# Audio-WestlakeU/FullSubNet

Measured on NVIDIA H100. Metric: frames_per_sec, higher is better.
Workload: dtype f16x3(hi+lo split, fp32-class)xf32acc

## Files before the change

### fullsubnet_b200/csrc/fsn_subband_tc.cu

```cuda
#include <cuda_fp16.h>
#include <stdlib.h>
#include <string.h>

#include "fsn_internal.cuh"
#include "fsn_tc_ptx.cuh"
#include "fsn_wgmma.cuh"

namespace fsn {
namespace tc {

using namespace ptx;

constexpr int NB = 32;
constexpr int KB = 64;
constexpr int KS = 32;
constexpr int US = 64;
constexpr int W_SUB = US * KS * 2;
constexpr int W_TILE = 4 * W_SUB;
constexpr int S_KBLK = NB * KB * 2;
constexpr int X_BLK = NB * KS * 2;
constexpr int MAX_STAGES = 4;
constexpr int MAX_MT = 3;
constexpr int OUT_T = 8;
constexpr int NTHREADS = 128 + 128 * MAX_MT;

struct PackedLayout {
  int H, MT, nkb0, nkb1, parts;
  size_t tiles0, tiles1;
  size_t off_bias, off_fcw, off_fcb, bytes;
};

__host__ __device__ inline PackedLayout packed_layout(int H, bool x3) {
  PackedLayout L;
  L.H = H; L.MT = H / 128;
  L.nkb0 = 1 + H / KS; L.nkb1 = 2 * H / KS;
  L.parts = x3 ? 2 : 1;
  L.tiles0 = (size_t)L.MT * L.nkb0 * L.parts;
  L.tiles1 = (size_t)L.MT * L.nkb1 * L.parts;
  L.off_bias = 2 * (L.tiles0 + L.tiles1) * W_TILE;
  L.off_fcw = L.off_bias + (size_t)2 * 4 * H * sizeof(float);
  L.off_fcb = L.off_fcw + (size_t)2 * H * sizeof(float);
  L.bytes = L.off_fcb + 256;
  return L;
}

__global__ void pack_kernel(const float* __restrict__ wih0, const float* __restrict__ whh0,
                            const float* __restrict__ wih1, const float* __restrict__ whh1,
                            const float* __restrict__ bih0, const float* __restrict__ bhh0,
                            const float* __restrict__ bih1, const float* __restrict__ bhh1,
                            const float* __restrict__ fcw, const float* __restrict__ fcb, int H, int Ksb, int x3,
                            int fc_out, uint8_t* __restrict__ out) {
  const PackedLayout L = packed_layout(H, x3 != 0);
  const size_t per_half = L.tiles0 + L.tiles1;
  const size_t total = 2 * per_half * 4 * US * 4;
  for (size_t i = blockIdx.x * (size_t)blockDim.x + threadIdx.x; i < total; i += (size_t)gridDim.x * blockDim.x) {
    const int c = (int)(i & 3);
    const int r = (int)((i >> 2) & (US - 1));
    const int g = (int)((i >> 8) & 3);
    const size_t st_abs = i >> 10;
    const int half = (int)(st_abs / per_half);
    size_t st = st_abs - half * per_half;
    const int layer = st >= L.tiles0;
    if (layer) st -= L.tiles0;
    const int part = (int)(st % L.parts);
    st /= L.parts;
    const int nkb = layer ? L.nkb1 : L.nkb0;
    const int kb = (int)(st % nkb);
    const int m = (int)(st / nkb);
    const int wrow = g * H + (half * L.MT + m) * US + r;
    __half v[8];
#pragma unroll
    for (int e = 0; e < 8; ++e) {
      const int kk = c * 8 + e;
      float w = 0.f;
      if (layer == 0) {
        if (kb == 0) { if (kk < Ksb) w = wih0[(size_t)wrow * Ksb + kk]; }
        else w = whh0[(size_t)wrow * H + (kb - 1) * KS + kk];
      } else {
        const int k = kb * KS + kk;
        w = (k < H) ? wih1[(size_t)wrow * H + k] : whh1[(size_t)wrow * H + (k - H)];
      }
      const __half hi = __float2half_rn(w);
      v[e] = part ? __float2half_rn(w - __half2float(hi)) : hi;
    }
    uint8_t* dst = out + st_abs * W_TILE + g * W_SUB + swz64_off(r, c * 8);
    *reinterpret_cast<uint4*>(dst) = *reinterpret_cast<const uint4*>(v);
  }
  float* bias = reinterpret_cast<float*>(out + L.off_bias);
  float* pfcw = reinterpret_cast<float*>(out + L.off_fcw);
  float* pfcb = reinterpret_cast<float*>(out + L.off_fcb);
  for (int i = blockIdx.x * blockDim.x + threadIdx.x; i < 4 * H; i += gridDim.x * blockDim.x) {
    bias[i] = bih0[i] + bhh0[i];
    bias[4 * H + i] = bih1[i] + bhh1[i];
  }
  for (int i = blockIdx.x * blockDim.x + threadIdx.x; i < 2 * H; i += gridDim.x * blockDim.x)
    pfcw[i] = (i < fc_out * H) ? fcw[i] : 0.f;
  if (blockIdx.x == 0 && threadIdx.x < 2) pfcb[threadIdx.x] = ((int)threadIdx.x < fc_out) ? fcb[threadIdx.x] : 0.f;
}

struct Smem {
  uint32_t w, x, h0, h1, lo, fcw, fcp, outst, rows, bars, total;
};
__host__ __device__ inline Smem smem_plan(int H, int stages, bool x3) {
  Smem s;
  const int nkh = H / KB;
  uint32_t o = 0;
  s.w = o; o += stages * W_TILE;
  s.x = o; o += 2 * X_BLK;
  s.h0 = o; o += 2 * nkh * S_KBLK;
  s.h1 = o; o += nkh * S_KBLK;
  s.lo = o; o += x3 ? (o - s.x) : 0;
  s.fcw = o; o += 4 * MAX_MT * 2 * NB * 4;
  s.fcp = o; o += 2 * 2 * NB * 4;
  s.outst = o; o += NB * 2 * OUT_T * 4;
  s.rows = o; o += NB * 16;
  s.bars = o; o += 256;
  s.total = o;
  return s;
}

struct Bars {
  uint64_t w_full[MAX_STAGES], w_empty[MAX_STAGES];
  uint64_t x_full[2], x_empty[2];
  uint64_t h0_ready[2], h0_empty[2];
  uint64_t h1_ready, h1_empty, fc_done;
  uint64_t l1_done;
  uint64_t fcp_full[2], fcp_empty[2];
  uint64_t turn[MAX_MT];
};
static_assert(sizeof(Bars) <= 256, "barrier block too large");

struct RowInfo {
  int src_b, src_f;
  float scale;
  int out_idx;
};

struct KArgs {
  const uint8_t* packed;
  const float* magT; const float* fbT; const float* inv2;
  const float* unit_scale;
  float* crm;
  int R, F, Tp, la, T, Ns, Nf, H, Ksb, act, Fsub, stages, cluster;
  int src_T, shrink;
  RowMap map;
  long long* stamps;
  int stamp_ctas, stamp_its;
};

enum ProbeField {
  PF_T_BEGIN = 0,
  PF_T_MMA0 = 1,
  PF_T_MMA1 = 2,
  PF_T_END = 3,
  PF_OPERAND = 4,
  PF_TURN = 5,
  PF_W_FULL = 6,
  PF_WAIT_GROUP = 7,
  PF_GROUP_LAT = 8,
  PF_STAGES = 9,
  PF_CELL = 10,
  PF_L1_DONE = 11,
  PF_H1_EMPTY = 12,
  PF_H0_EMPTY = 13,
  PF_FC_DONE = 14,
  PF_GT_BEGIN = 15,
  PROBE_FIELDS = 16
};
constexpr int PROBE_SLOTS = MAX_MT + 1;
static_assert(PROBE_FIELDS == FSN_SB_PROBE_FIELDS && PROBE_SLOTS == FSN_SB_PROBE_SLOTS,
              "probe record layout differs from fsn_b200.h (and fullsubnet_b200/_lib.py)");

__device__ __forceinline__ long long globaltimer() {
  uint64_t t;
  asm volatile("mov.u64 %0, %%globaltimer;" : "=l"(t));
  return (long long)t;
}

__device__ __forceinline__ float act_apply(float v, int act) {
  switch (act) {
    case FSN_ACT_RELU: return fmaxf(v, 0.f);
    case FSN_ACT_TANH: return tanhf(v);
    case FSN_ACT_RELU6: return fminf(fmaxf(v, 0.f), 6.f);
    default: return v;
  }
}
template <bool X3> __device__ __forceinline__ float sg(float x) { return X3 ? 1.0f / (1.0f + expf(-x)) : fast_sigmoid(x); }
template <bool X3> __device__ __forceinline__ float th(float x) { return X3 ? 1.0f - 2.0f / (1.0f + expf(2.0f * x)) : fast_tanh(x); }

__device__ __forceinline__ void release_stage(uint32_t bar, uint32_t pred, uint32_t local, uint32_t remote,
                                              uint32_t rank) {
  mbar_arrive_elect_if(bar, pred & local);
  mbar_arrive_remote_elect_if(bar, rank, pred & remote);
}

template <bool X3, bool PROBE>
__global__ void __launch_bounds__(NTHREADS, 1) sb_lstm_tc_kernel(const __grid_constant__ KArgs a) {
  constexpr int PARTS = X3 ? 2 : 1;
  long long pt = 0;
  auto mark = [&]() -> uint32_t {
    if constexpr (PROBE) {
      const long long n = clock64();
      const uint32_t d = (uint32_t)(n - pt);
      pt = n;
      return d;
    } else {
      return 0u;
    }
  };
  auto record = [&](int it, int layer, int slot) -> long long* {
    return a.stamps + ((((size_t)blockIdx.x * a.stamp_its + it) * 2 + layer) * PROBE_SLOTS + slot) * PROBE_FIELDS;
  };
  const bool probe_cta = PROBE && (int)blockIdx.x < a.stamp_ctas;
  extern __shared__ uint8_t smem_raw[];
  uint8_t* smem = smem_raw + ((1024u - (smem_u32(smem_raw) & 1023u)) & 1023u);
  const int H = a.H;
  const int MT = H / 128;
  const int nkh = H / KB;
  const int STAGES = a.stages;
  const int CL = a.cluster;
  const uint32_t cl_rank = cluster_ctarank();
  const int half = (int)(cl_rank & 1u);
  const uint32_t peer = cl_rank ^ 1u;
  const uint16_t cl_mask = (uint16_t)((0x55u & ((1u << (2 * CL)) - 1u)) << half);
  const Smem sp = smem_plan(H, STAGES, X3);
  const uint32_t LO = sp.lo - sp.x;
  const PackedLayout PL = packed_layout(H, X3);
  Bars& bars = *reinterpret_cast<Bars*>(smem + sp.bars);
  RowInfo* rows = reinterpret_cast<RowInfo*>(smem + sp.rows);
  float* fc_part = reinterpret_cast<float*>(smem + sp.fcw);
  float* fcp = reinterpret_cast<float*>(smem + sp.fcp);
  float* outst = reinterpret_cast<float*>(smem + sp.outst);
  const int warp = threadIdx.x >> 5, lane = threadIdx.x & 31;
  const int row0 = (blockIdx.x >> 1) * NB;
  const int Tp = a.Tp;

  if (threadIdx.x == 0) {
    for (int s = 0; s < STAGES; ++s) { mbar_init(&bars.w_full[s], 1); mbar_init(&bars.w_empty[s], CL); }
    for (int i = 0; i < 2; ++i) {
      mbar_init(&bars.x_full[i], 1); mbar_init(&bars.x_empty[i], 4 * MT);
      mbar_init(&bars.h0_ready[i], 5 * MT);
      mbar_init(&bars.h0_empty[i], MT);
      mbar_init(&bars.fcp_full[i], 1); mbar_init(&bars.fcp_empty[i], 1);
    }
    mbar_init(&bars.h1_ready, 5 * MT);
    mbar_init(&bars.h1_empty, MT);
    mbar_init(&bars.fc_done, 1);
    mbar_init(&bars.l1_done, 4 * MT);
    for (int m = 0; m < MAX_MT; ++m) mbar_init(&bars.turn[m], 4);
    asm volatile("fence.mbarrier_init.release.cluster;" ::: "memory");
  }
  if (threadIdx.x < NB) {
    RowInfo ri;
    const int r = row0 + threadIdx.x;
    ri.src_b = -1; ri.src_f = 0; ri.scale = 0.f; ri.out_idx = 0;
    if (r < a.R) {
      row_to_unit(a.map, r, ri.src_b, ri.src_f);
      ri.scale = a.inv2[ri.src_b];
      const int bq = r / a.Fsub, fq = r - bq * a.Fsub;
      ri.out_idx = bq * 2 * a.Fsub + fq;
    }
    rows[threadIdx.x] = ri;
  }
  {
    uint4* z = reinterpret_cast<uint4*>(smem + sp.x);
    const int n16 = (sp.fcw - sp.x) / 16;
    for (int i = threadIdx.x; i < n16; i += blockDim.x) z[i] = make_uint4(0, 0, 0, 0);
  }
  fence_proxy_async_smem();
  __syncthreads();
  cluster_sync_all();

  if (warp < 4) {
    asm volatile("setmaxnreg.dec.sync.aligned.u32 56;");
  if (warp == 0) {
    const uint8_t* stream = a.packed + (size_t)half * (PL.tiles0 + PL.tiles1) * W_TILE;
    uint32_t stage = 0, phase = 0;
    for (int it = 0; it <= Tp; ++it) {
      const size_t t_begin = (it < Tp) ? 0 : PL.tiles0;
      const size_t t_end = (it >= 1) ? PL.tiles0 + PL.tiles1 : PL.tiles0;
      const uint8_t* src = stream + t_begin * W_TILE;
      long long p_t0 = 0, p_g0 = 0;
      uint32_t p_empty = 0;
      if constexpr (PROBE) { p_g0 = globaltimer(); p_t0 = clock64(); pt = p_t0; }
      for (size_t tile = t_begin; tile < t_end; ++tile, src += W_TILE) {
        mark();
        mbar_wait_cta<false>(&bars.w_empty[stage], phase ^ 1);
        p_empty += mark();
        if (elect_one()) {
          mbar_expect_tx(&bars.w_full[stage], W_TILE);
          if (CL == 1) {
            bulk_g2s(smem + sp.w + stage * W_TILE, src, W_TILE, &bars.w_full[stage]);
          } else {
            const uint32_t slice = W_TILE / CL, off = (cl_rank >> 1) * slice;
            bulk_g2s_mc(smem + sp.w + stage * W_TILE + off, src + off, slice, &bars.w_full[stage], cl_mask);
          }
        }
        __syncwarp();
        if (++stage == (uint32_t)STAGES) { stage = 0; phase ^= 1; }
      }
      if (probe_cta && it < a.stamp_its && lane == 0) {
        long long* r = record(it, 0, MAX_MT);
        r[PF_T_BEGIN] = p_t0; r[PF_T_END] = clock64(); r[PF_OPERAND] = p_empty;
        r[PF_STAGES] = (long long)(t_end - t_begin); r[PF_GT_BEGIN] = p_g0;
      }
    }
  } else if (warp == 2) {
    const int nmag = 2 * a.Ns + 1;
    for (int t = 0; t < Tp; ++t) {
      mbar_wait_cta<true>(&bars.x_empty[t & 1], ((t >> 1) & 1) ^ 1);
      uint8_t* xb = smem + sp.x + (t & 1) * X_BLK;
      int f0 = t, f1 = t + 1;
      if (a.shrink > 1 && t > 0) { f0 = 1 + (t - 1) * a.shrink; f1 = min(f0 + a.shrink, a.src_T); }
      const float wmean = 1.0f / (float)(f1 - f0);
#pragma unroll 4
      for (int n = 0; n < NB; ++n) {
        const RowInfo ri = rows[n];
        float v = 0.f;
        if (ri.src_b >= 0 && lane < a.Ksb) {
          const int col = (lane < nmag) ? reflect_idx(ri.src_f + lane - a.Ns, a.F)
                                        : reflect_idx(ri.src_f + (lane - nmag) - a.Nf, a.F);
          const float* src = (lane < nmag) ? a.magT : a.fbT;
          if (a.shrink <= 1) {
            v = src[((size_t)ri.src_b * a.src_T + t) * a.F + col];
            v *= a.unit_scale ? a.unit_scale[(size_t)t * a.R + row0 + n] : ri.scale;
          } else {
            for (int fr = f0; fr < f1; ++fr) v += src[((size_t)ri.src_b * a.src_T + fr) * a.F + col];
            v *= wmean * (a.unit_scale ? a.unit_scale[(size_t)t * a.R + row0 + n] : ri.scale);
          }
        }
        const __half hi = __float2half_rn(v);
        *reinterpret_cast<__half*>(xb + swz64_off(n, lane)) = hi;
        if (X3) *reinterpret_cast<__half*>(xb + LO + swz64_off(n, lane)) = __float2half_rn(v - __half2float(hi));
      }
      fence_proxy_async_smem();
      __syncwarp();
      if (lane == 0) mbar_arrive(&bars.x_full[t & 1]);
    }
  } else if (warp == 3) {
    const float fcb0 = half ? 0.f : reinterpret_cast<const float*>(a.packed + PL.off_fcb)[0];
    const float fcb1 = half ? 0.f : reinterpret_cast<const float*>(a.packed + PL.off_fcb)[1];
    const RowInfo ri = rows[lane];
    int staged = 0, t_stage0 = 0;
    for (int t = 0; t < Tp; ++t) {
      mbar_wait_cta<true>(&bars.h1_ready, t & 1);
      float s0 = fcb0, s1 = fcb1;
      if (t >= a.la) {
        for (int w = 0; w < 4 * MT; ++w) {
          s0 += fc_part[(w * 2 + 0) * NB + lane];
          s1 += fc_part[(w * 2 + 1) * NB + lane];
        }
      }
      __syncwarp();
      if (lane == 0) mbar_arrive(&bars.fc_done);
      if (t < a.la) continue;
      const int u = t - a.la, b = u & 1;
      float* pb = fcp + b * 2 * NB;
      if (half) {
        mbar_wait<true>(&bars.fcp_empty[b], ((u >> 1) & 1) ^ 1);
        st_remote_f32(pb + lane, peer, s0);
        st_remote_f32(pb + NB + lane, peer, s1);
        __syncwarp();
        if (lane == 0) mbar_arrive_cluster(&bars.fcp_full[b], peer);
        continue;
      }
      mbar_wait<true>(&bars.fcp_full[b], (u >> 1) & 1);
      s0 += pb[lane];
      s1 += pb[NB + lane];
      __syncwarp();
      if (lane == 0) mbar_arrive_cluster(&bars.fcp_empty[b], peer);
      if (staged == 0) t_stage0 = u;
      outst[(lane * 2 + 0) * OUT_T + staged] = act_apply(s0, a.act);
      outst[(lane * 2 + 1) * OUT_T + staged] = act_apply(s1, a.act);
      ++staged;
      if (staged == OUT_T || t == Tp - 1) {
        if (ri.src_b >= 0) {
#pragma unroll
          for (int o = 0; o < 2; ++o) {
            float* dst = a.crm + ((size_t)ri.out_idx + (size_t)o * a.Fsub) * a.T + t_stage0;
            for (int i = 0; i < staged; ++i) dst[i] = outst[(lane * 2 + o) * OUT_T + i];
          }
        }
        staged = 0;
      }
    }
  }
  } else {
    asm volatile("setmaxnreg.inc.sync.aligned.u32 152;");
    const int m = __shfl_sync(0xffffffffu, (warp - 4) >> 2, 0);
    const int q = __shfl_sync(0xffffffffu, warp & 3, 0);
    const int s = half * MT + m;
    if (m < MT) {
      const float* bias_g = reinterpret_cast<const float*>(a.packed + PL.off_bias);
      const float* fcw = reinterpret_cast<const float*>(a.packed + PL.off_fcw);
      float* my_part = fc_part + (size_t)(warp - 4) * 2 * NB;
      float c0[16], c1[16];
#pragma unroll
      for (int i = 0; i < 16; ++i) c0[i] = c1[i] = 0.f;
      const uint32_t a_lo0 = wg::desc_lo(smem_u32(smem + sp.w));
      const uint32_t w_full0 = smem_u32(&bars.w_full[0]), w_empty0 = smem_u32(&bars.w_empty[0]);
      const uint32_t turn_next = smem_u32(&bars.turn[m + 1 < MT ? m + 1 : 0]);
      const uint32_t rel_local = CL == 1 && q == 0, rel_remote = CL > 1 && q < CL;
      const uint32_t rel_rank = 2 * q + half;
      int h0_seen = 0, h1_seen = 0, turns = 0;
      bool first_block = true;
      size_t tile_base = 0;
      for (int it = 0; it <= Tp; ++it) {
        for (int layer = 0; layer < 2; ++layer) {
          const int t = it - layer;
          if (t < 0 || t >= Tp) continue;
          long long p_t0 = 0, p_g0 = 0, p_mma0 = 0, p_mma1 = 0, p_commit = 0, p_commit_prev = 0;
          uint32_t p_opnd = 0, p_turn = 0, p_wfull = 0, p_wgw = 0, p_lat = 0, p_cell = 0, p_l1 = 0, p_h1e = 0, p_h0e = 0,
                   p_fc = 0;
          if constexpr (PROBE) { p_g0 = globaltimer(); p_t0 = clock64(); pt = p_t0; }
          if (layer == 0) {
            mbar_wait_cta<false>(&bars.x_full[t & 1], (t >> 1) & 1);
            for (; h0_seen < t; ++h0_seen) mbar_wait_cta<false>(&bars.h0_ready[h0_seen & 1], (h0_seen >> 1) & 1);
          } else {
            for (; h0_seen < t + 1; ++h0_seen) mbar_wait_cta<false>(&bars.h0_ready[h0_seen & 1], (h0_seen >> 1) & 1);
            for (; h1_seen < t; ++h1_seen) mbar_wait_cta<false>(&bars.h1_ready, h1_seen & 1);
          }
          p_opnd += mark();
          const uint32_t x_addr = smem_u32(smem + sp.x + (t & 1) * X_BLK);
          const uint32_t h0_cur = smem_u32(smem + sp.h0 + (t & 1) * nkh * S_KBLK);
          const uint32_t h0_prev = smem_u32(smem + sp.h0 + ((t + 1) & 1) * nkh * S_KBLK);
          const uint32_t h1_prev = smem_u32(smem + sp.h1);
          const int nkb = layer ? PL.nkb1 : PL.nkb0;
          const size_t first = tile_base + (layer ? ((it < Tp) ? PL.tiles0 : 0) : 0) + (size_t)m * nkb * PARTS;
          float acc[4][16];
#pragma unroll
          for (int g = 0; g < 4; ++g) {
#pragma unroll
            for (int i = 0; i < 16; ++i) acc[g][i] = 0.f;
            wg::fence_operand(acc[g]);
          }
          int prev_stage = -1;
          if (m > 0 || !first_block) { mbar_wait_cta<false>(&bars.turn[m], turns & 1); ++turns; }
          first_block = false;
          p_turn += mark();
          p_mma0 = pt;
          int stage = __shfl_sync(0xffffffffu, (int)(first % (size_t)STAGES), 0);
          uint32_t wphase = __shfl_sync(0xffffffffu, (uint32_t)((first / (size_t)STAGES) & 1), 0);
          auto issue_stage = [&](int part, uint32_t bd, uint32_t b_hi, uint32_t ends_block) {
            mark();
            mbar_wait_cta_warp(w_full0 + 8 * stage, wphase);
            p_wfull += mark();
            mbar_arrive_elect_if(turn_next, ends_block);
            wg::fence();
            const uint32_t ad = a_lo0 + stage * (W_TILE >> 4);
#pragma unroll
            for (int kk = 0; kk < 2; ++kk)
#pragma unroll
              for (int g = 0; g < 4; ++g) {
                const uint32_t a_off = g * (W_SUB >> 4) + kk * 2;
                wg::mma_f16_n32_w(acc[g], ad, a_off, wg::DESC_SW64_HI, bd, kk * 2, b_hi);
                if (X3 && part == 0) wg::mma_f16_n32_w(acc[g], ad, a_off, wg::DESC_SW64_HI, bd, (LO >> 4) + kk * 2, b_hi);
              }
            wg::commit();
            if constexpr (PROBE) p_commit = clock64();
            mark();
            wg::wait<1>();
            p_wgw += mark();
            if constexpr (PROBE) {
              if (prev_stage >= 0) p_lat += (uint32_t)(pt - p_commit_prev);
              p_commit_prev = p_commit;
            }
            release_stage(w_empty0 + 8 * prev_stage, prev_stage >= 0, rel_local, rel_remote, rel_rank);
            prev_stage = stage;
            if (++stage == STAGES) { stage = 0; wphase ^= 1; }
          };
          if (layer == 0) {
#pragma unroll
            for (int part = 0; part < PARTS; ++part) issue_stage(part, wg::desc_lo(x_addr), wg::DESC_SW64_HI, 0u);
          }
          const int nseg = layer ? 2 : 1;
          int seg = 0;
          do {
            uint32_t bd = wg::desc_lo(layer == 0 ? h0_prev : seg == 0 ? h0_cur : h1_prev);
            int kb = 0;
            do {
              const uint32_t ends_block = seg == nseg - 1 && kb == nkh - 1;
#pragma unroll
              for (int part = 0; part < PARTS; ++part) issue_stage(part, bd, wg::DESC_SW128_HI, 0u);
#pragma unroll
              for (int part = 0; part < PARTS; ++part)
                issue_stage(part, bd + (64 >> 4), wg::DESC_SW128_HI, part == PARTS - 1 ? ends_block : 0u);
              bd += S_KBLK >> 4;
            } while (++kb < nkh);
          } while (++seg < nseg);
          mark();
          wg::wait<0>();
#pragma unroll
          for (int g = 0; g < 4; ++g) wg::fence_operand(acc[g]);
          p_wgw += mark();
          if constexpr (PROBE) { p_lat += (uint32_t)(pt - p_commit_prev); p_mma1 = pt; }
          release_stage(w_empty0 + 8 * prev_stage, 1u, rel_local, rel_remote, rel_rank);
          if (lane == 0) mbar_arrive(layer ? &bars.l1_done : &bars.x_empty[t & 1]);
          if (layer == 1 && lane == 0) {
            if (q == 2) mbar_arrive_remote(&bars.h0_empty[t & 1], peer);
            if (q == 3) mbar_arrive_remote(&bars.h1_empty, peer);
          }
          p_cell += mark();
          if (layer == 1 && t >= 1) mbar_wait_cta<false>(&bars.fc_done, (t - 1) & 1);
          p_fc += mark();
          float fsum[2][8];
#pragma unroll
          for (int i = 0; i < 16; ++i) fsum[i >> 3][i & 7] = 0.f;
          __half hv[2][8];
          __half lv[2][8];
          uint8_t* hb = smem + (layer ? sp.h1 : sp.h0 + (t & 1) * nkh * S_KBLK) + s * S_KBLK;
#pragma unroll
          for (int hh = 0; hh < 2; ++hh) {
            const int u = s * US + 16 * q + (lane >> 2) + 8 * hh;
            const float* bl = bias_g + (layer ? 4 * H : 0);
            const float bi = bl[u], bff = bl[H + u], bg = bl[2 * H + u], bo = bl[3 * H + u];
            const float w0 = fcw[u], w1 = fcw[H + u];
#pragma unroll
            for (int j = 0; j < 4; ++j)
#pragma unroll
              for (int e = 0; e < 2; ++e) {
                const int ri = 4 * j + 2 * hh + e;
                const int ci = hh * 8 + j * 2 + e;
                const float cp = layer ? c1[ci] : c0[ci];
                const float cn = sg<X3>(acc[1][ri] + bff) * cp + sg<X3>(acc[0][ri] + bi) * th<X3>(acc[2][ri] + bg);
                if (layer) c1[ci] = cn; else c0[ci] = cn;
                const float h = sg<X3>(acc[3][ri] + bo) * th<X3>(cn);
                const __half hi = __float2half_rn(h);
                hv[hh][j * 2 + e] = hi;
                lv[hh][j * 2 + e] = __float2half_rn(h - __half2float(hi));
                if (layer) { fsum[0][j * 2 + e] += h * w0; fsum[1][j * 2 + e] += h * w1; }
              }
          }
          if (layer == 1) {
#pragma unroll
            for (int o = 0; o < 2; ++o)
#pragma unroll
              for (int r = 0; r < 8; ++r) {
                float v = fsum[o][r];
                v += __shfl_xor_sync(0xffffffffu, v, 4);
                v += __shfl_xor_sync(0xffffffffu, v, 8);
                v += __shfl_xor_sync(0xffffffffu, v, 16);
                fsum[o][r] = v;
              }
            if (lane < 4) {
#pragma unroll
              for (int o = 0; o < 2; ++o)
#pragma unroll
                for (int r = 0; r < 8; ++r) my_part[o * NB + 8 * (r >> 1) + 2 * lane + (r & 1)] = fsum[o][r];
            }
            p_cell += mark();
            mbar_wait_cta<false>(&bars.l1_done, t & 1);
            p_l1 += mark();
            mbar_wait_cta<false>(&bars.h1_empty, t & 1);
            p_h1e += mark();
          } else if (t >= 2) {
            p_cell += mark();
            mbar_wait_cta<false>(&bars.h0_empty[t & 1], ((t - 2) >> 1) & 1);
            p_h0e += mark();
          }
#pragma unroll
          for (int hh = 0; hh < 2; ++hh) {
            const int u = 16 * q + (lane >> 2) + 8 * hh;
            uint8_t* ub = hb + (u & 7) * 2;
            const int chunk = u >> 3;
#pragma unroll
            for (int j = 0; j < 4; ++j)
#pragma unroll
              for (int e = 0; e < 2; ++e) {
                const int n = 8 * j + 2 * (lane & 3) + e;
                uint8_t* p = ub + (n >> 3) * 1024 + (n & 7) * 128 + ((chunk ^ (n & 7)) << 4);
                *reinterpret_cast<__half*>(p) = hv[hh][j * 2 + e];
                if (X3) *reinterpret_cast<__half*>(p + LO) = lv[hh][j * 2 + e];
              }
          }
          fence_proxy_async_smem();
          __syncwarp();
          uint64_t* ready = layer ? &bars.h1_ready : &bars.h0_ready[t & 1];
          if (lane == 0) mbar_arrive(ready);
          named_sync(1 + m, 128);
          if (q == 0 && lane == 0) {
            mbar_arrive_expect_tx_remote(ready, peer, PARTS * S_KBLK);
            bulk_s2s_remote(hb, S_KBLK, ready, peer);
            if (X3) bulk_s2s_remote(hb + LO, S_KBLK, ready, peer);
          }
          if constexpr (PROBE) {
            p_cell += mark();
            if (probe_cta && it < a.stamp_its && q == 0 && lane == 0) {
              long long* r = record(it, layer, m);
              r[PF_T_BEGIN] = p_t0; r[PF_T_MMA0] = p_mma0; r[PF_T_MMA1] = p_mma1; r[PF_T_END] = pt;
              r[PF_OPERAND] = p_opnd; r[PF_TURN] = p_turn; r[PF_W_FULL] = p_wfull; r[PF_WAIT_GROUP] = p_wgw;
              r[PF_GROUP_LAT] = p_lat; r[PF_STAGES] = nkb * PARTS; r[PF_CELL] = p_cell; r[PF_L1_DONE] = p_l1;
              r[PF_H1_EMPTY] = p_h1e; r[PF_H0_EMPTY] = p_h0e; r[PF_FC_DONE] = p_fc; r[PF_GT_BEGIN] = p_g0;
            }
          }
        }
        tile_base += ((it < Tp) ? PL.tiles0 : 0) + ((it >= 1) ? PL.tiles1 : 0);
      }
    }
  }

  __syncthreads();
  cluster_sync_all();
}

}

static int sb_ksb(const fsn_model_desc* d) { return (2 * d->sb_num_neighbors + 1) + (2 * d->fb_num_neighbors + 1); }

static bool sb_tc_shape_ok(int H, int Ksb) { return H % 128 == 0 && H / 128 <= tc::MAX_MT && H >= 128 && Ksb <= tc::KS; }

bool sb_tc_supported(const fsn_model_desc* d) {
  if (d->cell_type != FSN_CELL_LSTM) return false;
  return sb_tc_shape_ok(d->sb_hidden, sb_ksb(d));
}

size_t sb_tc_packed_bytes_raw(int H, bool x3) { return tc::packed_layout(H, x3).bytes; }

size_t sb_tc_packed_bytes(const fsn_model_desc* d) {
  if (!sb_tc_supported(d)) return 0;
  return sb_tc_packed_bytes_raw(d->sb_hidden, d->precision == FSN_PREC_F16X3_TC);
}

int sb_tc_pack_raw(const fsn_seq_weights* sb, int H, int Ksb, int fc_out, void* packed, cudaStream_t st, bool x3) {
  FSN_REQUIRE(sb_tc_shape_ok(H, Ksb), FSN_ERR_UNSUPPORTED,
              "the fp16 tensor-core LSTM stack needs a hidden size in {128,256,384} and an input width <= 32");
  int dev = 0, sms = 132;
  cudaGetDevice(&dev);
  cudaDeviceGetAttribute(&sms, cudaDevAttrMultiProcessorCount, dev);
  tc::pack_kernel<<<sms * 4, 256, 0, st>>>(sb->w_ih[0], sb->w_hh[0], sb->w_ih[1], sb->w_hh[1], sb->b_ih[0], sb->b_hh[0],
                                           sb->b_ih[1], sb->b_hh[1], sb->fc_w, sb->fc_b, H, Ksb, x3 ? 1 : 0, fc_out,
                                           (uint8_t*)packed);
  FSN_CHECK_LAUNCH("sb pack_kernel");
  return FSN_OK;
}

int sb_tc_pack(const fsn_model_desc* d, const fsn_seq_weights* sb, void* packed, cudaStream_t st) {
  FSN_REQUIRE(sb_tc_supported(d), FSN_ERR_UNSUPPORTED,
              "FSN_PREC_F16_TC / FSN_PREC_F16X3_TC need sb_hidden in {128,256,384} and sub-band input width <= 32");
  return sb_tc_pack_raw(sb, d->sb_hidden, sb_ksb(d), 2, packed, st, d->precision == FSN_PREC_F16X3_TC);
}

template <bool X3, bool PROBE = false>
static int sb_tc_config(int H, int stages, int cluster, int pairs, cudaStream_t st, cudaLaunchConfig_t& cfg,
                        cudaLaunchAttribute* attr) {
  const tc::Smem sp = tc::smem_plan(H, stages, X3);
  const size_t smem = sp.total + 1024;
  int rc = check_cuda(cudaFuncSetAttribute(tc::sb_lstm_tc_kernel<X3, PROBE>, cudaFuncAttributeMaxDynamicSharedMemorySize,
                                           (int)smem), "sb_lstm_tc smem attr");
  if (rc) return rc;
// ... 145 lines not shown
```

### fullsubnet_b200/csrc/fsn_tc_ptx.cuh

```cuda
#pragma once
#include <cuda_fp16.h>
#include <stdint.h>
#include <stdio.h>

namespace fsn {
namespace ptx {

__device__ __forceinline__ uint32_t smem_u32(const void* p) { return (uint32_t)__cvta_generic_to_shared(p); }

__device__ __forceinline__ uint32_t cluster_ctarank() {
  uint32_t r;
  asm volatile("mov.u32 %0, %%cluster_ctarank;" : "=r"(r));
  return r;
}
__device__ __forceinline__ uint32_t mapa(uint32_t addr, uint32_t rank) {
  uint32_t r;
  asm volatile("mapa.shared::cluster.u32 %0, %1, %2;" : "=r"(r) : "r"(addr), "r"(rank));
  return r;
}
__device__ __forceinline__ void cluster_sync_all() {
  asm volatile("barrier.cluster.arrive.release.aligned;\n\tbarrier.cluster.wait.acquire.aligned;" ::: "memory");
}
__device__ __forceinline__ bool elect_one() {
  uint32_t pred;
  asm volatile(
      "{\n\t.reg .pred p;\n\t"
      "elect.sync _|p, 0xffffffff;\n\t"
      "selp.b32 %0, 1, 0, p;\n\t}"
      : "=r"(pred));
  return pred != 0;
}

__device__ __forceinline__ void mbar_init(uint64_t* bar, uint32_t count) {
  asm volatile("mbarrier.init.shared::cta.b64 [%0], %1;" ::"r"(smem_u32(bar)), "r"(count));
}
__device__ __forceinline__ void mbar_expect_tx(uint64_t* bar, uint32_t bytes) {
  asm volatile("mbarrier.arrive.expect_tx.shared::cta.b64 _, [%0], %1;" ::"r"(smem_u32(bar)), "r"(bytes) : "memory");
}
__device__ __forceinline__ void mbar_arrive_cluster(uint64_t* bar, uint32_t rank) {
  asm volatile("mbarrier.arrive.release.cluster.shared::cluster.b64 _, [%0];" ::"r"(mapa(smem_u32(bar), rank))
               : "memory");
}
__device__ __forceinline__ void mbar_arrive_cluster_relaxed(uint64_t* bar, uint32_t rank) {
  asm volatile("mbarrier.arrive.relaxed.cluster.shared::cluster.b64 _, [%0];" ::"r"(mapa(smem_u32(bar), rank))
               : "memory");
}
__device__ __forceinline__ void fence_release_cluster() { asm volatile("fence.acq_rel.cluster;" ::: "memory"); }
__device__ __forceinline__ bool mbar_try_wait(uint64_t* bar, uint32_t parity) {
  uint32_t ok;
  asm volatile(
      "{\n\t.reg .pred p;\n\t"
      "mbarrier.try_wait.parity.acquire.cluster.shared::cta.b64 p, [%1], %2;\n\t"
      "selp.b32 %0, 1, 0, p;\n\t}"
      : "=r"(ok)
      : "r"(smem_u32(bar)), "r"(parity)
      : "memory");
  return ok != 0;
}
__device__ __forceinline__ bool mbar_test_wait(uint64_t* bar, uint32_t parity) {
  uint32_t ok;
  asm volatile(
      "{\n\t.reg .pred p;\n\t"
      "mbarrier.test_wait.parity.acquire.cluster.shared::cta.b64 p, [%1], %2;\n\t"
      "selp.b32 %0, 1, 0, p;\n\t}"
      : "=r"(ok)
      : "r"(smem_u32(bar)), "r"(parity)
      : "memory");
  return ok != 0;
}
template <bool RELAXED>
__device__ __forceinline__ void mbar_wait(uint64_t* bar, uint32_t parity) {
  uint32_t spins = 0;
  while (!mbar_try_wait(bar, parity)) {
    if (RELAXED) __nanosleep(64);
    if (++spins > (RELAXED ? (1u << 24) : (1u << 27))) asm volatile("trap;");
  }
}

__device__ __forceinline__ void mbar_wait_mma(uint64_t* bar, uint32_t parity) {
  uint32_t spins = 0;
  while (!mbar_try_wait(bar, parity))
    if (++spins > (1u << 27)) asm volatile("trap;");
}

__device__ __forceinline__ bool mbar_try_wait_cta(uint64_t* bar, uint32_t parity) {
  uint32_t ok;
  asm volatile(
      "{\n\t.reg .pred p;\n\t"
      "mbarrier.try_wait.parity.acquire.cta.shared::cta.b64 p, [%1], %2;\n\t"
      "selp.b32 %0, 1, 0, p;\n\t}"
      : "=r"(ok)
      : "r"(smem_u32(bar)), "r"(parity)
      : "memory");
  return ok != 0;
}
template <bool SLEEP>
__device__ __forceinline__ void mbar_wait_cta(uint64_t* bar, uint32_t parity) {
  uint32_t spins = 0;
  while (!mbar_try_wait_cta(bar, parity)) {
    if (SLEEP) __nanosleep(64);
    if (++spins > (SLEEP ? (1u << 24) : (1u << 27))) asm volatile("trap;");
  }
}
__device__ __forceinline__ void mbar_wait_cta_warp(uint32_t bar, uint32_t parity) {
  asm volatile(
      "{\n\t.reg .pred p;\n\t.reg .b32 n;\n\t"
      "mov.b32 n, 0;\n"
      "WAIT:\n\t"
      "mbarrier.try_wait.parity.acquire.cta.shared::cta.b64 p, [%0], %1;\n\t"
      "vote.sync.all.pred p, p, 0xffffffff;\n\t"
      "@p bra.uni DONE;\n\t"
      "add.u32 n, n, 1;\n\t"
      "setp.gt.u32 p, n, 134217728;\n\t"
      "@p trap;\n\t"
      "bra.uni WAIT;\n"
      "DONE:\n\t}"
      ::"r"(bar), "r"(parity)
      : "memory");
}
__device__ __forceinline__ void mbar_arrive_elect_if(uint32_t bar, uint32_t pred) {
  asm volatile(
      "{\n\t.reg .pred e, p;\n\t"
      "elect.sync _|e, 0xffffffff;\n\t"
      "setp.ne.and.b32 p, %1, 0, e;\n\t"
      "@p mbarrier.arrive.shared::cta.b64 _, [%0];\n\t}"
      ::"r"(bar), "r"(pred)
      : "memory");
}
__device__ __forceinline__ void mbar_arrive_remote_elect_if(uint32_t bar, uint32_t rank, uint32_t pred) {
  asm volatile(
      "{\n\t.reg .pred e, p;\n\t.reg .b32 r;\n\t"
      "elect.sync _|e, 0xffffffff;\n\t"
      "setp.ne.and.b32 p, %2, 0, e;\n\t"
      "@p mapa.shared::cluster.u32 r, %0, %1;\n\t"
      "@p mbarrier.arrive.shared::cluster.b64 _, [r];\n\t}"
      ::"r"(bar), "r"(rank), "r"(pred)
      : "memory");
}
__device__ __forceinline__ void fence_proxy_async_smem() { asm volatile("fence.proxy.async.shared::cta;" ::: "memory"); }
__device__ __forceinline__ void mbar_arrive_remote(uint64_t* bar, uint32_t rank) {
  asm volatile("mbarrier.arrive.shared::cluster.b64 _, [%0];" ::"r"(mapa(smem_u32(bar), rank)) : "memory");
}
__device__ __forceinline__ void mbar_arrive_expect_tx_remote(uint64_t* bar, uint32_t rank, uint32_t bytes) {
  asm volatile("mbarrier.arrive.expect_tx.shared::cluster.b64 _, [%0], %1;" ::"r"(mapa(smem_u32(bar), rank)), "r"(bytes)
               : "memory");
}
__device__ __forceinline__ void bulk_s2s_remote(const void* src, uint32_t bytes, uint64_t* bar, uint32_t rank) {
  const uint32_t s = smem_u32(src);
  asm volatile("cp.async.bulk.shared::cluster.shared::cta.mbarrier::complete_tx::bytes [%0], [%1], %2, [%3];" ::"r"(
                   mapa(s, rank)),
               "r"(s), "r"(bytes), "r"(mapa(smem_u32(bar), rank))
               : "memory");
}
__device__ __forceinline__ void st_remote_f32(float* p, uint32_t rank, float v) {
  asm volatile("st.shared::cluster.f32 [%0], %1;" ::"r"(mapa(smem_u32(p), rank)), "f"(v) : "memory");
}
__device__ __forceinline__ void named_sync(uint32_t id, uint32_t count) {
  asm volatile("bar.sync %0, %1;" ::"r"(id), "r"(count) : "memory");
}

__device__ __forceinline__ void bulk_g2s(void* dst, const void* src, uint32_t bytes, uint64_t* bar) {
  asm volatile("cp.async.bulk.shared::cluster.global.mbarrier::complete_tx::bytes [%0], [%1], %2, [%3];" ::"r"(
                   smem_u32(dst)),
               "l"(src), "r"(bytes), "r"(smem_u32(bar))
               : "memory");
}
__device__ __forceinline__ void bulk_g2s_mc(void* dst, const void* src, uint32_t bytes, uint64_t* bar, uint16_t mask) {
  asm volatile(
      "cp.async.bulk.shared::cluster.global.mbarrier::complete_tx::bytes.multicast::cluster [%0], [%1], %2, [%3], %4;" ::"r"(
          smem_u32(dst)),
      "l"(src), "r"(bytes), "r"(smem_u32(bar)), "h"(mask)
      : "memory");
}
__device__ __forceinline__ void tma_load_2d(void* dst, const void* tmap, int c0, int c1, uint64_t* bar) {
  asm volatile(
      "cp.async.bulk.tensor.2d.shared::cluster.global.mbarrier::complete_tx::bytes [%0], [%1, {%2, %3}], [%4];" ::"r"(
          smem_u32(dst)),
      "l"(tmap), "r"(c0), "r"(c1), "r"(smem_u32(bar))
      : "memory");
}
__device__ __forceinline__ void fence_proxy_async() { asm volatile("fence.proxy.async;" ::: "memory"); }

__device__ __forceinline__ void mbar_arrive(uint64_t* bar) {
  asm volatile("mbarrier.arrive.shared::cta.b64 _, [%0];" ::"r"(smem_u32(bar)) : "memory");
}
__host__ __device__ __forceinline__ int swz128_off(int row, int k) {
  return (row >> 3) * 1024 + (row & 7) * 128 + ((((k >> 3) ^ (row & 7)) & 7) << 4) + (k & 7) * 2;
}
__host__ __device__ __forceinline__ int swz64_off(int row, int k) {
  return (row >> 3) * 512 + (row & 7) * 64 + ((((k >> 3) ^ ((row >> 1) & 3)) & 3) << 4) + (k & 7) * 2;
}

__device__ __forceinline__ float fast_sigmoid(float x) { return __fdividef(1.0f, 1.0f + __expf(-x)); }
__device__ __forceinline__ float fast_tanh(float x) { return 1.0f - __fdividef(2.0f, 1.0f + __expf(2.0f * x)); }

}
}
```

### fullsubnet_b200/csrc/fsn_wgmma.cuh

```cuda
#pragma once
#include <stdint.h>

namespace fsn {
namespace wg {

__device__ __forceinline__ void fence() { asm volatile("wgmma.fence.sync.aligned;" ::: "memory"); }
__device__ __forceinline__ void commit() { asm volatile("wgmma.commit_group.sync.aligned;" ::: "memory"); }
template <int N>
__device__ __forceinline__ void wait() { asm volatile("wgmma.wait_group.sync.aligned %0;" ::"n"(N) : "memory"); }
template <int R>
__device__ __forceinline__ void fence_operand(float (&d)[R]) {
#pragma unroll
  for (int i = 0; i < R; ++i) asm volatile("" : "+f"(d[i])::"memory");
}

__device__ __forceinline__ uint64_t desc_sw128(uint32_t saddr) {
  return (uint64_t)((saddr >> 4) & 0x3FFF) | (1ull << 16) | (64ull << 32) | (1ull << 62);
}
__device__ __forceinline__ uint64_t desc_sw64(uint32_t saddr) {
  return (uint64_t)((saddr >> 4) & 0x3FFF) | (1ull << 16) | (32ull << 32) | (2ull << 62);
}

__device__ __forceinline__ void mma_f16_n16(float (&d)[8], uint64_t a, uint64_t b, uint32_t scale_d) {
  asm volatile(
      "{\n\t.reg .pred p;\n\tsetp.ne.b32 p, %10, 0;\n\t"
      "wgmma.mma_async.sync.aligned.m64n16k16.f32.f16.f16 {%0,%1,%2,%3,%4,%5,%6,%7}, %8, %9, p, 1, 1, 0, 0;\n\t}"
      : "+f"(d[0]), "+f"(d[1]), "+f"(d[2]), "+f"(d[3]), "+f"(d[4]), "+f"(d[5]), "+f"(d[6]), "+f"(d[7])
      : "l"(a), "l"(b), "r"(scale_d)
      : "memory");
}

__device__ __forceinline__ void mma_f16_n32(float (&d)[16], uint64_t a, uint64_t b, uint32_t scale_d) {
  asm volatile(
      "{\n\t.reg .pred p;\n\tsetp.ne.b32 p, %18, 0;\n\t"
      "wgmma.mma_async.sync.aligned.m64n32k16.f32.f16.f16 {%0,%1,%2,%3,%4,%5,%6,%7,%8,%9,%10,%11,%12,%13,%14,%15}, %16, %17, p, 1, 1, 0, 0;\n\t}"
      : "+f"(d[0]), "+f"(d[1]), "+f"(d[2]), "+f"(d[3]), "+f"(d[4]), "+f"(d[5]), "+f"(d[6]), "+f"(d[7]), "+f"(d[8]), "+f"(d[9]), "+f"(d[10]), "+f"(d[11]), "+f"(d[12]), "+f"(d[13]), "+f"(d[14]), "+f"(d[15])
      : "l"(a), "l"(b), "r"(scale_d)
      : "memory");
}

constexpr uint32_t DESC_SW128_HI = 64u | (1u << 30), DESC_SW64_HI = 32u | (2u << 30);
__device__ __forceinline__ uint32_t desc_lo(uint32_t saddr) { return ((saddr >> 4) & 0x3FFF) | (1u << 16); }

__device__ __forceinline__ void mma_f16_n32_w(float (&d)[16], uint32_t a_lo, uint32_t a_off, uint32_t a_hi,
                                              uint32_t b_lo, uint32_t b_off, uint32_t b_hi) {
  asm volatile(
      "{\n\t.reg .b32 al, bl;\n\t.reg .b64 a, b;\n\t"
      "add.u32 al, %16, %17;\n\tadd.u32 bl, %19, %20;\n\t"
      "mov.b64 a, {al, %18};\n\tmov.b64 b, {bl, %21};\n\t"
      "wgmma.mma_async.sync.aligned.m64n32k16.f32.f16.f16 {%0,%1,%2,%3,%4,%5,%6,%7,%8,%9,%10,%11,%12,%13,%14,%15}, a, b, 1, 1, 1, 0, 0;\n\t}"
      : "+f"(d[0]), "+f"(d[1]), "+f"(d[2]), "+f"(d[3]), "+f"(d[4]), "+f"(d[5]), "+f"(d[6]), "+f"(d[7]), "+f"(d[8]), "+f"(d[9]), "+f"(d[10]), "+f"(d[11]), "+f"(d[12]), "+f"(d[13]), "+f"(d[14]), "+f"(d[15])
      : "r"(a_lo), "r"(a_off), "r"(a_hi), "r"(b_lo), "r"(b_off), "r"(b_hi)
      : "memory");
}

__device__ __forceinline__ void mma_f16_n64(float (&d)[32], uint64_t a, uint64_t b, uint32_t scale_d) {
  asm volatile(
      "{\n\t.reg .pred p;\n\tsetp.ne.b32 p, %34, 0;\n\t"
      "wgmma.mma_async.sync.aligned.m64n64k16.f32.f16.f16 {%0,%1,%2,%3,%4,%5,%6,%7,%8,%9,%10,%11,%12,%13,%14,%15,%16,%17,%18,%19,%20,%21,%22,%23,%24,%25,%26,%27,%28,%29,%30,%31}, %32, %33, p, 1, 1, 0, 0;\n\t}"
      : "+f"(d[0]), "+f"(d[1]), "+f"(d[2]), "+f"(d[3]), "+f"(d[4]), "+f"(d[5]), "+f"(d[6]), "+f"(d[7]), "+f"(d[8]), "+f"(d[9]), "+f"(d[10]), "+f"(d[11]), "+f"(d[12]), "+f"(d[13]), "+f"(d[14]), "+f"(d[15]), "+f"(d[16]), "+f"(d[17]), "+f"(d[18]), "+f"(d[19]), "+f"(d[20]), "+f"(d[21]), "+f"(d[22]), "+f"(d[23]), "+f"(d[24]), "+f"(d[25]), "+f"(d[26]), "+f"(d[27]), "+f"(d[28]), "+f"(d[29]), "+f"(d[30]), "+f"(d[31])
      : "l"(a), "l"(b), "r"(scale_d)
      : "memory");
}

__device__ __forceinline__ void mma_f16_n128(float (&d)[64], uint64_t a, uint64_t b, uint32_t scale_d) {
  asm volatile(
      "{\n\t.reg .pred p;\n\tsetp.ne.b32 p, %66, 0;\n\t"
      "wgmma.mma_async.sync.aligned.m64n128k16.f32.f16.f16 {%0,%1,%2,%3,%4,%5,%6,%7,%8,%9,%10,%11,%12,%13,%14,%15,%16,%17,%18,%19,%20,%21,%22,%23,%24,%25,%26,%27,%28,%29,%30,%31,%32,%33,%34,%35,%36,%37,%38,%39,%40,%41,%42,%43,%44,%45,%46,%47,%48,%49,%50,%51,%52,%53,%54,%55,%56,%57,%58,%59,%60,%61,%62,%63}, %64, %65, p, 1, 1, 0, 0;\n\t}"
      : "+f"(d[0]), "+f"(d[1]), "+f"(d[2]), "+f"(d[3]), "+f"(d[4]), "+f"(d[5]), "+f"(d[6]), "+f"(d[7]), "+f"(d[8]), "+f"(d[9]), "+f"(d[10]), "+f"(d[11]), "+f"(d[12]), "+f"(d[13]), "+f"(d[14]), "+f"(d[15]), "+f"(d[16]), "+f"(d[17]), "+f"(d[18]), "+f"(d[19]), "+f"(d[20]), "+f"(d[21]), "+f"(d[22]), "+f"(d[23]), "+f"(d[24]), "+f"(d[25]), "+f"(d[26]), "+f"(d[27]), "+f"(d[28]), "+f"(d[29]), "+f"(d[30]), "+f"(d[31]), "+f"(d[32]), "+f"(d[33]), "+f"(d[34]), "+f"(d[35]), "+f"(d[36]), "+f"(d[37]), "+f"(d[38]), "+f"(d[39]), "+f"(d[40]), "+f"(d[41]), "+f"(d[42]), "+f"(d[43]), "+f"(d[44]), "+f"(d[45]), "+f"(d[46]), "+f"(d[47]), "+f"(d[48]), "+f"(d[49]), "+f"(d[50]), "+f"(d[51]), "+f"(d[52]), "+f"(d[53]), "+f"(d[54]), "+f"(d[55]), "+f"(d[56]), "+f"(d[57]), "+f"(d[58]), "+f"(d[59]), "+f"(d[60]), "+f"(d[61]), "+f"(d[62]), "+f"(d[63])
      : "l"(a), "l"(b), "r"(scale_d)
      : "memory");
}

__device__ __forceinline__ void mma_tf32_n128(float (&d)[64], uint64_t a, uint64_t b, uint32_t scale_d) {
  asm volatile(
      "{\n\t.reg .pred p;\n\tsetp.ne.b32 p, %66, 0;\n\t"
      "wgmma.mma_async.sync.aligned.m64n128k8.f32.tf32.tf32 {%0,%1,%2,%3,%4,%5,%6,%7,%8,%9,%10,%11,%12,%13,%14,%15,%16,%17,%18,%19,%20,%21,%22,%23,%24,%25,%26,%27,%28,%29,%30,%31,%32,%33,%34,%35,%36,%37,%38,%39,%40,%41,%42,%43,%44,%45,%46,%47,%48,%49,%50,%51,%52,%53,%54,%55,%56,%57,%58,%59,%60,%61,%62,%63}, %64, %65, p, 1, 1;\n\t}"
      : "+f"(d[0]), "+f"(d[1]), "+f"(d[2]), "+f"(d[3]), "+f"(d[4]), "+f"(d[5]), "+f"(d[6]), "+f"(d[7]), "+f"(d[8]), "+f"(d[9]), "+f"(d[10]), "+f"(d[11]), "+f"(d[12]), "+f"(d[13]), "+f"(d[14]), "+f"(d[15]), "+f"(d[16]), "+f"(d[17]), "+f"(d[18]), "+f"(d[19]), "+f"(d[20]), "+f"(d[21]), "+f"(d[22]), "+f"(d[23]), "+f"(d[24]), "+f"(d[25]), "+f"(d[26]), "+f"(d[27]), "+f"(d[28]), "+f"(d[29]), "+f"(d[30]), "+f"(d[31]), "+f"(d[32]), "+f"(d[33]), "+f"(d[34]), "+f"(d[35]), "+f"(d[36]), "+f"(d[37]), "+f"(d[38]), "+f"(d[39]), "+f"(d[40]), "+f"(d[41]), "+f"(d[42]), "+f"(d[43]), "+f"(d[44]), "+f"(d[45]), "+f"(d[46]), "+f"(d[47]), "+f"(d[48]), "+f"(d[49]), "+f"(d[50]), "+f"(d[51]), "+f"(d[52]), "+f"(d[53]), "+f"(d[54]), "+f"(d[55]), "+f"(d[56]), "+f"(d[57]), "+f"(d[58]), "+f"(d[59]), "+f"(d[60]), "+f"(d[61]), "+f"(d[62]), "+f"(d[63])
      : "l"(a), "l"(b), "r"(scale_d)
      : "memory");
}

__device__ __forceinline__ void mma_tf32_n256(float (&d)[128], uint64_t a, uint64_t b, uint32_t scale_d) {
  asm volatile(
      "{\n\t.reg .pred p;\n\tsetp.ne.b32 p, %130, 0;\n\t"
      "wgmma.mma_async.sync.aligned.m64n256k8.f32.tf32.tf32 {%0,%1,%2,%3,%4,%5,%6,%7,%8,%9,%10,%11,%12,%13,%14,%15,%16,%17,%18,%19,%20,%21,%22,%23,%24,%25,%26,%27,%28,%29,%30,%31,%32,%33,%34,%35,%36,%37,%38,%39,%40,%41,%42,%43,%44,%45,%46,%47,%48,%49,%50,%51,%52,%53,%54,%55,%56,%57,%58,%59,%60,%61,%62,%63,%64,%65,%66,%67,%68,%69,%70,%71,%72,%73,%74,%75,%76,%77,%78,%79,%80,%81,%82,%83,%84,%85,%86,%87,%88,%89,%90,%91,%92,%93,%94,%95,%96,%97,%98,%99,%100,%101,%102,%103,%104,%105,%106,%107,%108,%109,%110,%111,%112,%113,%114,%115,%116,%117,%118,%119,%120,%121,%122,%123,%124,%125,%126,%127}, %128, %129, p, 1, 1;\n\t}"
      : "+f"(d[0]), "+f"(d[1]), "+f"(d[2]), "+f"(d[3]), "+f"(d[4]), "+f"(d[5]), "+f"(d[6]), "+f"(d[7]), "+f"(d[8]), "+f"(d[9]), "+f"(d[10]), "+f"(d[11]), "+f"(d[12]), "+f"(d[13]), "+f"(d[14]), "+f"(d[15]), "+f"(d[16]), "+f"(d[17]), "+f"(d[18]), "+f"(d[19]), "+f"(d[20]), "+f"(d[21]), "+f"(d[22]), "+f"(d[23]), "+f"(d[24]), "+f"(d[25]), "+f"(d[26]), "+f"(d[27]), "+f"(d[28]), "+f"(d[29]), "+f"(d[30]), "+f"(d[31]), "+f"(d[32]), "+f"(d[33]), "+f"(d[34]), "+f"(d[35]), "+f"(d[36]), "+f"(d[37]), "+f"(d[38]), "+f"(d[39]), "+f"(d[40]), "+f"(d[41]), "+f"(d[42]), "+f"(d[43]), "+f"(d[44]), "+f"(d[45]), "+f"(d[46]), "+f"(d[47]), "+f"(d[48]), "+f"(d[49]), "+f"(d[50]), "+f"(d[51]), "+f"(d[52]), "+f"(d[53]), "+f"(d[54]), "+f"(d[55]), "+f"(d[56]), "+f"(d[57]), "+f"(d[58]), "+f"(d[59]), "+f"(d[60]), "+f"(d[61]), "+f"(d[62]), "+f"(d[63]), "+f"(d[64]), "+f"(d[65]), "+f"(d[66]), "+f"(d[67]), "+f"(d[68]), "+f"(d[69]), "+f"(d[70]), "+f"(d[71]), "+f"(d[72]), "+f"(d[73]), "+f"(d[74]), "+f"(d[75]), "+f"(d[76]), "+f"(d[77]), "+f"(d[78]), "+f"(d[79]), "+f"(d[80]), "+f"(d[81]), "+f"(d[82]), "+f"(d[83]), "+f"(d[84]), "+f"(d[85]), "+f"(d[86]), "+f"(d[87]), "+f"(d[88]), "+f"(d[89]), "+f"(d[90]), "+f"(d[91]), "+f"(d[92]), "+f"(d[93]), "+f"(d[94]), "+f"(d[95]), "+f"(d[96]), "+f"(d[97]), "+f"(d[98]), "+f"(d[99]), "+f"(d[100]), "+f"(d[101]), "+f"(d[102]), "+f"(d[103]), "+f"(d[104]), "+f"(d[105]), "+f"(d[106]), "+f"(d[107]), "+f"(d[108]), "+f"(d[109]), "+f"(d[110]), "+f"(d[111]), "+f"(d[112]), "+f"(d[113]), "+f"(d[114]), "+f"(d[115]), "+f"(d[116]), "+f"(d[117]), "+f"(d[118]), "+f"(d[119]), "+f"(d[120]), "+f"(d[121]), "+f"(d[122]), "+f"(d[123]), "+f"(d[124]), "+f"(d[125]), "+f"(d[126]), "+f"(d[127])
      : "l"(a), "l"(b), "r"(scale_d)
      : "memory");
}

}
}
```

Baseline: 127,200.

## Load hi weight tiles into registers via ldmatrix for split-precision WGMMA and release stages early

For the x3 hi/lo path, the shared A weight tile of part 0 is now loaded into registers with ldmatrix and reused for both the hi and lo B operands through register-sourced WGMMA. The work is split into four commit groups so the stage's weight buffer can be released to the producer and cluster peers as soon as the registers are loaded, before the MMAs retire. The empty barrier count becomes 4x to match the new per-group arrivals. This aims to cut shared-memory descriptor re-reads of A and shorten how long weight stages stay occupied, at the cost of extra register pressure, more commit/wait points and a more intricate barrier protocol.

```diff
diff --git a/fullsubnet_b200/csrc/fsn_subband_tc.cu b/fullsubnet_b200/csrc/fsn_subband_tc.cu
--- a/fullsubnet_b200/csrc/fsn_subband_tc.cu
+++ b/fullsubnet_b200/csrc/fsn_subband_tc.cu
@@ -5,6 +5,8 @@
 #include "fsn_internal.cuh"
 #include "fsn_tc_ptx.cuh"
 #include "fsn_wgmma.cuh"
+
+#include <type_traits>
 
 namespace fsn {
 namespace tc {
@@ -188,10 +190,16 @@
 template <bool X3> __device__ __forceinline__ float sg(float x) { return X3 ? 1.0f / (1.0f + expf(-x)) : fast_sigmoid(x); }
 template <bool X3> __device__ __forceinline__ float th(float x) { return X3 ? 1.0f - 2.0f / (1.0f + expf(2.0f * x)) : fast_tanh(x); }
 
+template <int N>
 __device__ __forceinline__ void release_stage(uint32_t bar, uint32_t pred, uint32_t local, uint32_t remote,
                                               uint32_t rank) {
-  mbar_arrive_elect_if(bar, pred & local);
-  mbar_arrive_remote_elect_if(bar, rank, pred & remote);
+  if constexpr (N == 1) {
+    mbar_arrive_elect_if(bar, pred & local);
+    mbar_arrive_remote_elect_if(bar, rank, pred & remote);
+  } else {
+    mbar_arrive_n_elect_if<N>(bar, pred & local);
+    mbar_arrive_remote_n_elect_if<N>(bar, rank, pred & remote);
+  }
 }
 
 template <bool X3, bool PROBE>
@@ -236,7 +244,7 @@
   const int Tp = a.Tp;
 
   if (threadIdx.x == 0) {
-    for (int s = 0; s < STAGES; ++s) { mbar_init(&bars.w_full[s], 1); mbar_init(&bars.w_empty[s], CL); }
+    for (int s = 0; s < STAGES; ++s) { mbar_init(&bars.w_full[s], 1); mbar_init(&bars.w_empty[s], X3 ? 4 * CL : CL); }
     for (int i = 0; i < 2; ++i) {
       mbar_init(&bars.x_full[i], 1); mbar_init(&bars.x_empty[i], 4 * MT);
       mbar_init(&bars.h0_ready[i], 5 * MT);
@@ -398,9 +406,11 @@
 #pragma unroll
       for (int i = 0; i < 16; ++i) c0[i] = c1[i] = 0.f;
       const uint32_t a_lo0 = wg::desc_lo(smem_u32(smem + sp.w));
+      const uint32_t a_ldsm0 = smem_u32(smem + sp.w) + swz64_off(16 * q + 8 * ((lane >> 3) & 1) + (lane & 7), 8 * (lane >> 4));
       const uint32_t w_full0 = smem_u32(&bars.w_full[0]), w_empty0 = smem_u32(&bars.w_empty[0]);
       const uint32_t turn_next = smem_u32(&bars.turn[m + 1 < MT ? m + 1 : 0]);
       const uint32_t rel_local = CL == 1 && q == 0, rel_remote = CL > 1 && q < CL;
+      const uint32_t grp_local = CL == 1, grp_n = CL > 1 ? CL : 0;
       const uint32_t rel_rank = 2 * q + half;
       int h0_seen = 0, h1_seen = 0, turns = 0;
       bool first_block = true;
@@ -441,32 +451,59 @@
           p_mma0 = pt;
           int stage = __shfl_sync(0xffffffffu, (int)(first % (size_t)STAGES), 0);
           uint32_t wphase = __shfl_sync(0xffffffffu, (uint32_t)((first / (size_t)STAGES) & 1), 0);
+          auto retire_prev = [&](auto pending) {
+            if constexpr (PROBE) p_commit = clock64();
+            mark();
+            wg::wait<decltype(pending)::value>();
+            p_wgw += mark();
+            if constexpr (PROBE) {
+              if (prev_stage >= 0) p_lat += (uint32_t)(pt - p_commit_prev);
+              p_commit_prev = p_commit;
+            }
+            release_stage<X3 ? 4 : 1>(w_empty0 + 8 * prev_stage, prev_stage >= 0, rel_local, rel_remote, rel_rank);
+          };
           auto issue_stage = [&](int part, uint32_t bd, uint32_t b_hi, uint32_t ends_block) {
             mark();
             mbar_wait_cta_warp(w_full0 + 8 * stage, wphase);
             p_wfull += mark();
             mbar_arrive_elect_if(turn_next, ends_block);
-            wg::fence();
-            const uint32_t ad = a_lo0 + stage * (W_TILE >> 4);
-#pragma unroll
-            for (int kk = 0; kk < 2; ++kk)
-#pragma unroll
-              for (int g = 0; g < 4; ++g) {
-                const uint32_t a_off = g * (W_SUB >> 4) + kk * 2;
-                wg::mma_f16_n32_w(acc[g], ad, a_off, wg::DESC_SW64_HI, bd, kk * 2, b_hi);
-                if (X3 && part == 0) wg::mma_f16_n32_w(acc[g], ad, a_off, wg::DESC_SW64_HI, bd, (LO >> 4) + kk * 2, b_hi);
+            if (X3 && part == 0) {
+              const uint32_t la = a_ldsm0 + stage * W_TILE;
+              uint32_t wa[3][2][4];
+#pragma unroll
+              for (int grp = 0; grp < 4; ++grp) {
+                const int kk = grp >> 1, g0 = 2 * (grp & 1);
+                uint32_t (&w)[2][4] = wa[grp % 3];
+#pragma unroll
+                for (int i = 0; i < 2; ++i) ldsm_x4(w[i], (la ^ (kk * 32)) + (g0 + i) * W_SUB);
+                wg::fence();
+                if (grp == 3) mbar_arrive_group_elect(w_empty0 + 8 * stage, grp_local, half, grp_n);
+#pragma unroll
+                for (int i = 0; i < 2; ++i) {
+                  wg::mma_f16_n32_rs_w(acc[g0 + i], w[i], bd, kk * 2, b_hi);
+                  wg::mma_f16_n32_rs_w(acc[g0 + i], w[i], bd, (LO >> 4) + kk * 2, b_hi);
+                }
+                wg::commit();
+                if (grp == 1) {
+                  retire_prev(std::integral_constant<int, 2>{});
+                } else if (grp == 2) {
+                  mark();
+                  wg::wait<2>();
+                  p_wgw += mark();
+                }
               }
-            wg::commit();
-            if constexpr (PROBE) p_commit = clock64();
-            mark();
-            wg::wait<1>();
-            p_wgw += mark();
-            if constexpr (PROBE) {
-              if (prev_stage >= 0) p_lat += (uint32_t)(pt - p_commit_prev);
-              p_commit_prev = p_commit;
+            } else {
+              wg::fence();
+              const uint32_t ad = a_lo0 + stage * (W_TILE >> 4);
+#pragma unroll
+              for (int kk = 0; kk < 2; ++kk)
+#pragma unroll
+                for (int g = 0; g < 4; ++g)
+                  wg::mma_f16_n32_w(acc[g], ad, g * (W_SUB >> 4) + kk * 2, wg::DESC_SW64_HI, bd, kk * 2, b_hi);
+              wg::commit();
+              retire_prev(std::integral_constant<int, 1>{});
             }
-            release_stage(w_empty0 + 8 * prev_stage, prev_stage >= 0, rel_local, rel_remote, rel_rank);
-            prev_stage = stage;
+            prev_stage = (X3 && part == 0) ? -1 : stage;
             if (++stage == STAGES) { stage = 0; wphase ^= 1; }
           };
           if (layer == 0) {
@@ -494,7 +531,7 @@
           for (int g = 0; g < 4; ++g) wg::fence_operand(acc[g]);
           p_wgw += mark();
           if constexpr (PROBE) { p_lat += (uint32_t)(pt - p_commit_prev); p_mma1 = pt; }
-          release_stage(w_empty0 + 8 * prev_stage, 1u, rel_local, rel_remote, rel_rank);
+          release_stage<X3 ? 4 : 1>(w_empty0 + 8 * prev_stage, 1u, rel_local, rel_remote, rel_rank);
           if (lane == 0) mbar_arrive(layer ? &bars.l1_done : &bars.x_empty[t & 1]);
           if (layer == 1 && lane == 0) {
             if (q == 2) mbar_arrive_remote(&bars.h0_empty[t & 1], peer);
diff --git a/fullsubnet_b200/csrc/fsn_tc_ptx.cuh b/fullsubnet_b200/csrc/fsn_tc_ptx.cuh
--- a/fullsubnet_b200/csrc/fsn_tc_ptx.cuh
+++ b/fullsubnet_b200/csrc/fsn_tc_ptx.cuh
@@ -137,6 +137,51 @@
       ::"r"(bar), "r"(rank), "r"(pred)
       : "memory");
 }
+template <int N>
+__device__ __forceinline__ void mbar_arrive_n_elect_if(uint32_t bar, uint32_t pred) {
+  asm volatile(
+      "{\n\t.reg .pred e, p;\n\t"
+      "elect.sync _|e, 0xffffffff;\n\t"
+      "setp.ne.and.b32 p, %1, 0, e;\n\t"
+      "@p mbarrier.arrive.shared::cta.b64 _, [%0], %2;\n\t}"
+      ::"r"(bar), "r"(pred), "n"(N)
+      : "memory");
+}
+template <int N>
+__device__ __forceinline__ void mbar_arrive_remote_n_elect_if(uint32_t bar, uint32_t rank, uint32_t pred) {
+  asm volatile(
+      "{\n\t.reg .pred e, p;\n\t.reg .b32 r;\n\t"
+      "elect.sync _|e, 0xffffffff;\n\t"
+      "setp.ne.and.b32 p, %2, 0, e;\n\t"
+      "@p mapa.shared::cluster.u32 r, %0, %1;\n\t"
+      "@p mbarrier.arrive.shared::cluster.b64 _, [r], %3;\n\t}"
+      ::"r"(bar), "r"(rank), "r"(pred), "n"(N)
+      : "memory");
+}
+__device__ __forceinline__ void mbar_arrive_group_elect(uint32_t bar, uint32_t local, uint32_t base, uint32_t n) {
+  asm volatile(
+      "{\n\t.reg .pred e, p;\n\t.reg .b32 r, k;\n\t"
+      "elect.sync _|e, 0xffffffff;\n\t"
+      "setp.ne.and.b32 p, %1, 0, e;\n\t"
+      "@p mbarrier.arrive.shared::cta.b64 _, [%0];\n\t"
+      "setp.gt.and.u32 p, %3, 0, e;\n\t"
+      "@p mapa.shared::cluster.u32 r, %0, %2;\n\t"
+      "@p mbarrier.arrive.shared::cluster.b64 _, [r];\n\t"
+      "setp.gt.and.u32 p, %3, 1, e;\n\t"
+      "add.u32 k, %2, 2;\n\t"
+      "@p mapa.shared::cluster.u32 r, %0, k;\n\t"
+      "@p mbarrier.arrive.shared::cluster.b64 _, [r];\n\t"
+      "setp.gt.and.u32 p, %3, 2, e;\n\t"
+      "add.u32 k, %2, 4;\n\t"
+      "@p mapa.shared::cluster.u32 r, %0, k;\n\t"
+      "@p mbarrier.arrive.shared::cluster.b64 _, [r];\n\t"
+      "setp.gt.and.u32 p, %3, 3, e;\n\t"
+      "add.u32 k, %2, 6;\n\t"
+      "@p mapa.shared::cluster.u32 r, %0, k;\n\t"
+      "@p mbarrier.arrive.shared::cluster.b64 _, [r];\n\t}"
+      ::"r"(bar), "r"(local), "r"(base), "r"(n)
+      : "memory");
+}
 __device__ __forceinline__ void fence_proxy_async_smem() { asm volatile("fence.proxy.async.shared::cta;" ::: "memory"); }
 __device__ __forceinline__ void mbar_arrive_remote(uint64_t* bar, uint32_t rank) {
   asm volatile("mbarrier.arrive.shared::cluster.b64 _, [%0];" ::"r"(mapa(smem_u32(bar), rank)) : "memory");
@@ -191,6 +236,13 @@
   return (row >> 3) * 512 + (row & 7) * 64 + ((((k >> 3) ^ ((row >> 1) & 3)) & 3) << 4) + (k & 7) * 2;
 }
 
+__device__ __forceinline__ void ldsm_x4(uint32_t (&r)[4], uint32_t saddr) {
+  asm volatile("ldmatrix.sync.aligned.m8n8.x4.shared.b16 {%0,%1,%2,%3}, [%4];"
+               : "=r"(r[0]), "=r"(r[1]), "=r"(r[2]), "=r"(r[3])
+               : "r"(saddr)
+               : "memory");
+}
+
 __device__ __forceinline__ float fast_sigmoid(float x) { return __fdividef(1.0f, 1.0f + __expf(-x)); }
 __device__ __forceinline__ float fast_tanh(float x) { return 1.0f - __fdividef(2.0f, 1.0f + __expf(2.0f * x)); }
 
diff --git a/fullsubnet_b200/csrc/fsn_wgmma.cuh b/fullsubnet_b200/csrc/fsn_wgmma.cuh
--- a/fullsubnet_b200/csrc/fsn_wgmma.cuh
+++ b/fullsubnet_b200/csrc/fsn_wgmma.cuh
@@ -54,6 +54,18 @@
       : "memory");
 }
 
+__device__ __forceinline__ void mma_f16_n32_rs_w(float (&d)[16], const uint32_t (&a)[4], uint32_t b_lo, uint32_t b_off,
+                                                 uint32_t b_hi) {
+  asm volatile(
+      "{\n\t.reg .b32 bl;\n\t.reg .b64 b;\n\t"
+      "add.u32 bl, %20, %21;\n\t"
+      "mov.b64 b, {bl, %22};\n\t"
+      "wgmma.mma_async.sync.aligned.m64n32k16.f32.f16.f16 {%0,%1,%2,%3,%4,%5,%6,%7,%8,%9,%10,%11,%12,%13,%14,%15}, {%16,%17,%18,%19}, b, 1, 1, 1, 0;\n\t}"
+      : "+f"(d[0]), "+f"(d[1]), "+f"(d[2]), "+f"(d[3]), "+f"(d[4]), "+f"(d[5]), "+f"(d[6]), "+f"(d[7]), "+f"(d[8]), "+f"(d[9]), "+f"(d[10]), "+f"(d[11]), "+f"(d[12]), "+f"(d[13]), "+f"(d[14]), "+f"(d[15])
+      : "r"(a[0]), "r"(a[1]), "r"(a[2]), "r"(a[3]), "r"(b_lo), "r"(b_off), "r"(b_hi)
+      : "memory");
+}
+
 __device__ __forceinline__ void mma_f16_n64(float (&d)[32], uint64_t a, uint64_t b, uint32_t scale_d) {
   asm volatile(
       "{\n\t.reg .pred p;\n\tsetp.ne.b32 p, %34, 0;\n\t"
```

New measurement: 128,200 (median of 6 runs). No clear change (+0.9%).
